# zhoupengwei/tloam

Hardware: AMD Instinct MI355X
Metric: gauss_newton_iters_per_sec (higher is better)
Workload: dtype f64

## Files before the change

tloam_amd/csrc/tl_api.hip:

```cpp
#include "tl_ctx.hpp"

using namespace tl;

extern "C" {

int tloam_abi_version(void) { return TLOAM_ABI_VERSION; }

const char* tloam_status_string(int s) {
  switch (s) {
    case TLOAM_OK: return "ok";
    case TLOAM_E_INVALID: return "invalid argument";
    case TLOAM_E_TOO_FEW_POINTS: return "fewer than 10 points in a feature cloud";
    case TLOAM_E_BAD_POSE: return "predicted pose is not a rigid transform";
    case TLOAM_E_HIP: return "HIP error / no gfx950 device";
    case TLOAM_E_RCCL: return "RCCL error";
    case TLOAM_E_NOT_READY: return "call sequence violated";
    case TLOAM_E_WEIGHT_RANGE: return "GNC weight outside [0,1]";
    default: return "unknown status";
  }
}

void tloam_default_config(tloam_tls_config* c) {
  if (!c) return;
  memset(c, 0, sizeof(*c));
// ... 29 lines not shown
  if (const char* e = getenv("TLOAM_DEBUG_MAX_SWEEPS")) c->dbg_max_sweeps = atoi(e);
  c->dbg_no_build_reuse = getenv("TLOAM_NO_BUILD_REUSE") != nullptr;
  c->dbg_no_eval_reuse = getenv("TLOAM_NO_EVAL_REUSE") != nullptr;
  c->no_device_loop = getenv("TLOAM_NO_DEVICE_LOOP") != nullptr;
  c->no_persistent_solve = getenv("TLOAM_NO_PERSISTENT_SOLVE") != nullptr;
  c->no_grid_ahead = getenv("TLOAM_NO_GRID_AHEAD") != nullptr;
  c->no_direct_set = getenv("TLOAM_NO_DIRECT_SET") != nullptr;
  c->no_qbin_ride = getenv("TLOAM_NO_QBIN_RIDE") != nullptr;
  if (const char* e = getenv("TLOAM_DEBUG_FAIL_HANDOVER")) c->dbg_fail_handover = atoi(e);
  {
    int cus = 0;
    if (hipDeviceGetAttribute(&cus, hipDeviceAttributeMultiprocessorCount, device_id) != hipSuccess) cus = 0;
    c->device_cus = cus;
  }
  c->fused_large = getenv("TLOAM_FUSED_LARGE") != nullptr;
  if (const char* e = getenv("TLOAM_PLANNED_SWEEPS")) c->dbg_planned_sweeps = atoi(e);
  memset(&c->stats, 0, sizeof(c->stats));
  constexpr size_t kBoxDoubles = (size_t)kKinds * 64 * 6 + 8;
  const unsigned flags = hipHostMallocMapped | hipHostMallocCoherent;
  const bool up = hipStreamCreateWithFlags(&c->stream, hipStreamNonBlocking) == hipSuccess &&
                  c->h_state.alloc(kMirrorSlots, flags) == hipSuccess && c->h_small.alloc(4096, hipHostMallocDefault) == hipSuccess &&
                  c->h_mirror.alloc(kMirrorSlots, flags) == hipSuccess && ((uintptr_t)c->h_mirror.h & 63u) == 0 &&
                  c->h_mirror.map() == hipSuccess && c->h_bbox.alloc(kBoxDoubles, flags) == hipSuccess &&
                  c->h_bbox.map() == hipSuccess && c->h_fault.alloc(kFaultWords, flags) == hipSuccess &&
                  c->h_fault.map() == hipSuccess;
  if (up) {
    c->h_state.zero();
    c->h_mirror.zero();
    c->h_bbox.zero();
    c->h_fault.zero();
  }
  if (!up || ensure_common(c) != TLOAM_OK) {
    (void)hipGetLastError();
    tloam_destroy(c);
    return TLOAM_E_HIP;
  }
  (void)hipMemsetAsync(c->state.p, 0, sizeof(GnState), c->stream);
  (void)hipMemsetAsync(c->seg_n.p, 0, 8 * sizeof(int), c->stream);
  (void)hipStreamSynchronize(c->stream);
  *out = c;
  return TLOAM_OK;
}

void tloam_destroy(tloam_ctx* c) {
  if (!c) return;
  (void)hipSetDevice(c->device);
  if (c->stream) (void)hipStreamSynchronize(c->stream);
  tlh::comm_release(c);
  tlh::loop_release(c);
  for (auto& e : c->ev_pool) (void)hipEventDestroy(e);
  for (hipEvent_t e : c->stage_ev)
    if (e) (void)hipEventDestroy(e);
// ... 81 lines not shown
```

tloam_amd/csrc/tl_api_frames.hip:

```cpp
#include <chrono>
#include "tl_ctx.hpp"

using namespace tl;

namespace tlh {
int wait_word(tloam_ctx* c, const unsigned long long* p, unsigned long long seq) {
  for (unsigned spins = 1;; ++spins) {
    if (__atomic_load_n(p, __ATOMIC_ACQUIRE) == seq) return TLOAM_OK;
    if ((spins & 0x7ffu) == 0) {
      const hipError_t e = hipStreamQuery(c->stream);
      if (e == hipSuccess) return __atomic_load_n(p, __ATOMIC_ACQUIRE) == seq ? TLOAM_OK : 1;
      if (e != hipErrorNotReady) HIPC(c, e);
    }
    __builtin_ia32_pause();
  }
}
int wait_segment(tloam_ctx* c, const unsigned long long* seg, unsigned long long number, unsigned long long payload[7]) {
  const unsigned long long seq = check_mix(number);
  for (unsigned spins = 1;; ++spins) {
    unsigned long long w[8], x = 0ull;
    for (int i = 0; i < 8; ++i) { w[i] = __atomic_load_n(seg + i, __ATOMIC_ACQUIRE); x ^= i < 7 ? tl::seg_word(w[i], i) : w[i]; }
    if (x == seq) {
      for (int i = 0; i < 7; ++i) payload[i] = w[i];
      return TLOAM_OK;
// ... 209 lines not shown
      const int rc = reserve_query_sort(c, out);
      if (rc != TLOAM_OK) return rc;
      frame->qbin->tile_of_slot = c->tile_of_slot.p;
      frame->qbin->rank_in_tile = c->tile_fill.p;
      frame->qbin->tile_cnt = c->tile_cnt.p;
      if (frame->fi.tile_cnt == c->tile_cnt.p) { qbin = frame->qbin; frame->qbin_done = true; }
    }
    launch_grid_scan_finalize_scatter_1p(gs, G.cell_cnt.p, nc + 1, G.cell_start.p, G.scan1p.p, c->h_fault.dev + kFaultScan1p, G.cell_of_pt.p,
                                         G.rank_of_pt.p, G.gp.p, c->stream, qbin, out);
    return TLOAM_OK;
  }
  const int tiles = scan_tiles_only(G.cell_cnt.p, G.cell_scan.p, nc + 1, G.scan_tmp.p, c->stream);
  if (tiles > 0) {
    launch_grid_finalize_scatter_all(gs, G.cell_scan.p, G.scan_tmp.p, tiles, G.cell_start.p, G.cell_cnt.p, G.cell_of_pt.p,
                                     G.rank_of_pt.p, G.gp.p, c->stream);
  } else {
    launch_exclusive_scan_u64(G.cell_cnt.p, G.cell_scan.p, nc + 1, G.scan_tmp.p, c->stream);
    launch_grid_finalize_all(gs, G.cell_scan.p, G.cell_start.p, G.cell_cnt.p, c->stream);
    launch_grid_scatter_all(gs, G.cell_of_pt.p, G.cell_scan.p, G.rank_of_pt.p, G.gp.p, c->stream);
  }
  return TLOAM_OK;
}
int build_grids(tloam_ctx* c, GridBuffers& G, const double radius[kKinds], GridView out[kKinds], FrameInitHook* frame) {
  CloudRef clouds[kKinds];
  bool known = true;
  for (int k = 0; k < kKinds; ++k) {
    const KindData& K = c->kd[k];
    clouds[k] = CloudRef{K.tx.p, K.ty.p, K.tz.p, K.tgt_set ? K.n_tgt : 0};
    if (radius[k] > 0.0 && clouds[k].n > 0 && !c->tgt_box_valid[k]) known = false;
  }
  return build_grids_over(c, G, radius, clouds, out, known ? c->tgt_box : nullptr, frame);
}
int enqueue_target_bounds(tloam_ctx* c) {
  GridSet gs;
  memset(&gs, 0, sizeof(gs));
  for (int k = 0; k < kKinds; ++k) {
    const KindData& K = c->kd[k];
    gs.tx[k] = K.tx.p; gs.ty[k] = K.ty.p; gs.tz[k] = K.tz.p;
    gs.n[k] = K.tgt_set ? (int)K.n_tgt : 0;
  }
  launch_bbox_all(gs, c->h_bbox.dev, c->stream);
  return TLOAM_OK;
}
void finish_target_bounds(tloam_ctx* c) {
  reduce_box_rows(c->h_bbox, c->tgt_box);
  for (int k = 0; k < kKinds; ++k) c->tgt_box_valid[k] = c->kd[k].tgt_set && c->kd[k].n_tgt > 0;
}
void exchange_clouds(tloam_ctx* c, FrameClouds& F) {
  for (int k = 0; k < kKinds; ++k) {
    KindData& K = c->kd[k];
    std::swap(K.n_src_full, F.n_src_full[k]); std::swap(K.src_lo, F.src_lo[k]); std::swap(K.n_src, F.n_src[k]);
    std::swap(K.n_tgt, F.n_tgt[k]);
    std::swap(K.src_aos, F.src_aos[k]); std::swap(K.tgt_aos, F.tgt_aos[k]);
    std::swap(K.src_ptr, F.src_ptr[k]);
    std::swap(K.tx, F.tx[k]); std::swap(K.ty, F.ty[k]); std::swap(K.tz, F.tz[k]);
    std::swap(K.src_set, F.src_set[k]); std::swap(K.tgt_set, F.tgt_set[k]);
    for (int a = 0; a < 6; ++a) std::swap(c->tgt_box[k][a], F.tgt_box[k][a]);
    std::swap(c->tgt_box_valid[k], F.tgt_box_valid[k]);
    K.grid_valid = false;
  }
  c->grids_ahead = false; c->tgt_gen++;
  std::swap(c->src_pack, F.src_pack);
  c->have_build = false;
}
int source_frame_reserve(tloam_ctx* c, const size_t n[4], size_t cnt4[4]) {
  size_t lo4[kKinds], hi4[kKinds];
  tloam_shard_ranges_frame(n, c->rank, c->nranks, lo4, hi4);
  for (int k = 0; k < kKinds; ++k) {
    KindData& K = c->kd[k];
// ... 65 lines not shown
  K.tgt_set = true;
  return TLOAM_OK;
}
}

int tloam_set_source(tloam_ctx* c, int kind, const double* xyz, size_t n) {
  if (!c) return TLOAM_E_INVALID;
  HIPC(c, hipSetDevice(c->device));
  const int rc = set_source_async(c, kind, xyz, n);
  if (rc != TLOAM_OK) return rc;
  HIPC(c, hipStreamSynchronize(c->stream));
  return TLOAM_OK;
}

int tloam_set_target(tloam_ctx* c, int kind, const double* xyz, size_t n) {
  if (!c) return TLOAM_E_INVALID;
  HIPC(c, hipSetDevice(c->device));
  return tlh::set_target_copy(c, kind, xyz, n, hipMemcpyHostToDevice);
}

int tloam_set_source_frame(tloam_ctx* c, const double* const xyz[4], const size_t n[4]) {
  if (!c || !xyz || !n) return TLOAM_E_INVALID;
  HIPC(c, hipSetDevice(c->device));
  return set_source_frame_packed(c, xyz, n);
}

int tloam_set_target_frame(tloam_ctx* c, const double* const xyz[4], const size_t n[4]) {
  if (!c || !xyz || !n) return TLOAM_E_INVALID;
  for (int k = 0; k < kKinds; ++k)
    if ((n[k] > 0 && !xyz[k]) || n[k] > kMaxPoints) return TLOAM_E_INVALID;
  HIPC(c, hipSetDevice(c->device));
  return tlh::set_target_frame_from(c, xyz, n, hipMemcpyHostToDevice);
}
}

namespace tlh {
int set_target_frame_from(tloam_ctx* c, const double* const xyz[4], const size_t n[4], hipMemcpyKind from) {
  int rc = TLOAM_OK;
  for (int k = 0; k < kKinds && rc == TLOAM_OK; ++k) rc = set_target_async(c, k, xyz[k], n[k], false, from);
  if (rc == TLOAM_OK) {
    IngestArgs A;
    for (int k = 0; k < kKinds; ++k) {
      KindData& K = c->kd[k];
      A.aos[k] = K.tgt_aos.p; A.x[k] = K.tx.p; A.y[k] = K.ty.p; A.z[k] = K.tz.p;
      A.n[k] = (int)K.n_tgt;
    }
    launch_ingest_targets(A, c->h_bbox.dev, c->stream);
  }
  HIPC(c, hipStreamSynchronize(c->stream));
  if (rc == TLOAM_OK) finish_target_bounds(c);
  if (rc == TLOAM_OK && one_rank(c) && !c->no_grid_ahead) {
    double radius[kKinds];
    GridView views[kKinds];
    bool all = true;
    for (int k = 0; k < kKinds; ++k) { radius[k] = kind_radius(c->cfg, k); all = all && c->tgt_box_valid[k]; }
    if (all) {
      rc = build_grids(c, c->grids_next, radius, views, nullptr);
      if (rc == TLOAM_OK) {
        for (int k = 0; k < kKinds; ++k) c->gv_next[k] = views[k];
        c->grids_ahead = true;
        c->grids_next_gen = c->tgt_gen;
      }
    }
  }
  return rc;
}
}

extern "C" {

int tloam_frame_stash(tloam_ctx* c, int slot) {
  if (!c || slot < 0 || slot > (1 << 20)) return TLOAM_E_INVALID;
  if (c->active) return TLOAM_E_NOT_READY;
  HIPC(c, hipSetDevice(c->device));
  if ((size_t)slot >= c->frame_store.size()) c->frame_store.resize((size_t)slot + 1);
  if (c->frame_selected == slot) {
    exchange_clouds(c, *c->frame_store[slot]);
    c->frame_selected = -1;
    return TLOAM_OK;
  }
  if (c->frame_selected >= 0) return TLOAM_E_NOT_READY;
  if (!c->frame_store[slot]) {
    c->frame_store[slot].reset(new (std::nothrow) FrameClouds());
    if (!c->frame_store[slot]) return TLOAM_E_INVALID;
  } else {
    HIPC(c, hipStreamSynchronize(c->stream));
    *c->frame_store[slot] = FrameClouds();
  }
// ... 28 lines not shown
```

tloam_amd/csrc/tl_api_match.hip:

```cpp
#include <atomic>
#include <chrono>

#include "tl_ctx.hpp"

using namespace tl;

namespace {
int sync_stream(tloam_ctx* c) {
  HIPC(c, hipStreamSynchronize(c->stream));
  return TLOAM_OK;
}
}

namespace tlh {
int reserve_seg(tloam_ctx* c, int k, size_t n) {
  KindData& K = c->kd[k];
  const size_t cap = round_up(std::max<size_t>(n, 1), kChunk) + kChunk;
  HIPC(c, K.c_idx.reserve(cap));
  if (cap > K.c_stride) {
    const size_t stride = std::max(cap, K.c_stride + K.c_stride / 2);
    HIPC(c, K.c_buf.reserve(stride * kSegStreams));
    K.c_stride = stride;
  }
  K.c_cap = cap - kChunk;
// ... 352 lines not shown
    GridView gviews[kKinds];
    for (int k = 0; k < kKinds; ++k) gviews[k] = c->kd[k].gv;
    const size_t ntiles = (size_t)build_tile_count(gviews, c->sv.slot_off);
    HIPC(c, c->tile_cnt.reserve(ntiles + 1 > c->tile_cnt.cap ? 2 * ntiles + 64 : ntiles + 1));
    hook.fi.tile_cnt = c->tile_cnt.p;
    hook.fi.n_tile_cnt = (int)ntiles + 1;
    launch_frame_init(hook.fi, hook.b, c->stream);
  }
  if (c->direct) {
    bool all = true;
    for (int k = 0; k < kKinds; ++k) all = all && c->kd[k].gv.n > 0;
    if (!all) {
      c->direct = false;
      HIPC(c, hipMemsetAsync(c->seg_n.p, 0, kKinds * sizeof(int), c->stream));
    }
  }
  c->wait_us = 0.0;
  c->mu = 1.0;
  c->noise_bound_sq = c->cfg.noise_bound * c->cfg.noise_bound;
  if (c->noise_bound_sq < 1e-16) c->noise_bound_sq = 1e-2;
  for (int k = 0; k < kKinds; ++k) { c->prev_cost[k] = INFINITY; c->cur_cost[k] = INFINITY; }
  c->iter = 0;
  c->active = true;
  c->have_build = false;
  memset(&c->stats, 0, sizeof(c->stats));
  memcpy(c->stats.se3, x, sizeof(x));
  c->ev_used = 0;
  c->ev_batch_idx.clear();
  c->batch_launches = 0;
  return TLOAM_OK;
}

namespace {
constexpr int kMaxOuterFast = kMirrorSlots;

void outer_params(const tloam_ctx* c, BuildParams* bp, GridView grids[kKinds]) {
  for (int k = 0; k < kKinds; ++k) {
    bp->radius[k] = kind_radius(c->cfg, k);
    bp->maxnum[k] = kind_maxnum(c->cfg, k);
    bp->active[k] = kind_active(c->cfg, k);
    grids[k] = c->kd[k].gv;
  }
  bp->edge_dir_thres = c->cfg.edge_dir_thres;
}
int outer_reserve(tloam_ctx* c, const GridView grids[kKinds]) { return tlh::reserve_query_sort(c, grids); }
}
// ... 1046 lines not shown
```

tloam_amd/csrc/tl_api_submap.hip:

```cpp
#include "tl_ctx.hpp"

using namespace tl;

extern "C" {

void tloam_submap_default_config(tloam_submap_config* cfg) {
  if (!cfg) return;
  cfg->planar_frame_size = 3;
  cfg->sphere_frame_size = 3;
  cfg->edge_crop_box_length = 100.0;
  cfg->ground_crop_box_length = 100.0;
  cfg->edge_down_sample_submap = 0.3;
  cfg->ground_down_sample_submap = 0.45;
  cfg->ground_down_sample = 0.3;
}

namespace {
int submap_reserve_work(tloam_ctx* c, size_t n) {
  SubmapState& S = c->submap;
  const size_t m = std::max<size_t>(n, 1), cap = voxel_table_size(m);
  HIPC(c, S.min_partial.reserve(256 * 6)); HIPC(c, S.vmin.reserve(8)); HIPC(c, S.counts.reserve(8));
  if (!S.overflow.p) {
    HIPC(c, S.overflow.reserve(8));
    HIPC(c, hipMemsetAsync(S.overflow.p, 0, 8 * sizeof(int), c->stream));
// ... 34 lines not shown
  J.mask = voxel_table_size(std::max<size_t>(n, 1)) - 1;
  W.min_partial = S.min_partial.p; W.vmin = S.vmin.p;
  W.keys = S.keys.p; W.cnt = S.cnt.p; W.off = S.off.p;
  W.slot_of_pt = S.slot_of_pt.p; W.urank = S.urank.p; W.members = S.members.p; W.sorted = S.sorted.p;
  W.leader = S.leader.p; W.leader_scan = S.leader_scan.p; W.scan_tmp = S.scan_tmp.p; W.overflow = S.overflow.p;
  W.n_out = S.counts.p;
  W.host_seg = &c->h_mirror.dev[kMirrorSlots - 1].w[0];
  W.host_seq = ++c->mirror_seq;
  W.use_ticket = (c->vox_ticket || (long long)(n + 256) / 256 > (long long)vox_emit_resident_blocks(c->device_cus)) ? 1 : 0;
  W.fault = c->h_fault.dev + kFaultVoxEmit;
  S.pending_seq = W.host_seq;
  *Jout = J;
  *Wout = W;
  return TLOAM_OK;
}
int submap_crop_voxel(tloam_ctx* c, const CropVoxelSeg seg[2], int nseg) {
  VoxelJob J;
  VoxelWork W;
  const int rc = submap_job(c, seg, nseg, &J, &W);
  if (rc != TLOAM_OK) return rc;
  launch_crop_voxel(J, W, c->stream);
  return TLOAM_OK;
}
int submap_upload(tloam_ctx* c, const double* xyz, size_t n, hipMemcpyKind from = hipMemcpyHostToDevice) {
  SubmapState& S = c->submap;
  HIPC(c, S.in_aos.reserve(3 * std::max<size_t>(n, 1)));
  if (n > 0) HIPC(c, hipMemcpyAsync(S.in_aos.p, xyz, sizeof(double) * 3 * n, from, c->stream));
  return TLOAM_OK;
}
int submap_finish(tloam_ctx* c, size_t* n_edge, size_t* n_ground) {
  SubmapState& S = c->submap;
  unsigned long long h[2] = {0, 0};
  int ov = 0;
  bool have = false;
  if (S.pending_seq) {
    const unsigned long long* seg = &c->h_mirror[kMirrorSlots - 1].w[0];
    unsigned long long pay[7];
    const int rc = wait_segment(c, seg, S.pending_seq, pay);
    if (rc < 0) return rc;
    if (rc == TLOAM_OK) { h[0] = pay[0]; h[1] = pay[1]; ov = (int)pay[2]; have = true; }
    S.pending_seq = 0ull;
  }
  if (!have) {
    HIPC(c, hipMemcpyAsync(h, S.counts.p, sizeof(h), hipMemcpyDeviceToHost, c->stream));
    HIPC(c, hipMemcpyAsync(&ov, S.overflow.p, sizeof(int), hipMemcpyDeviceToHost, c->stream));
    HIPC(c, hipStreamSynchronize(c->stream));
// ... 16 lines not shown
  if (!c || (n_planar && !planar) || (n_sphere && !sphere) || (n_edge && !edge) || (n_ground && !ground) ||
      n_planar > kMaxPoints || n_sphere > kMaxPoints || n_edge > kMaxPoints || n_ground > kMaxPoints)
    return TLOAM_E_INVALID;
  HIPC(c, hipSetDevice(c->device));
  const tloam_submap_config want = cfg_or_default(cfg, tloam_submap_default_config);
  if (!tlh::submap_config_ok(want))
    return TLOAM_E_INVALID;
  return tlh::submap_init_body(c, want, planar, n_planar, sphere, n_sphere, edge, n_edge, ground, n_ground, hipMemcpyHostToDevice);
}

}

namespace tlh {
bool submap_config_ok(const tloam_submap_config& want) {
  return want.planar_frame_size >= 1 && want.sphere_frame_size >= 1 && want.edge_down_sample_submap > 0.0 &&
         want.ground_down_sample_submap > 0.0 && want.ground_down_sample > 0.0;
}

int submap_init_body(tloam_ctx* c, const tloam_submap_config& want, const double* planar, size_t n_planar, const double* sphere,
                     size_t n_sphere, const double* edge, size_t n_edge, const double* ground, size_t n_ground, hipMemcpyKind from) {
  SubmapState& S = c->submap;
  S = SubmapState();
  S.cfg = want;
  int rc = set_target_copy(c, TLOAM_KIND_EDGE, edge, n_edge, from);
  if (rc == TLOAM_OK) rc = set_target_copy(c, TLOAM_KIND_PLANAR, planar, n_planar, from);
  if (rc == TLOAM_OK) rc = set_target_copy(c, TLOAM_KIND_SPHERE, sphere, n_sphere, from);
  if (rc != TLOAM_OK) return rc;
  rc = submap_upload(c, ground, n_ground, from);
  if (rc != TLOAM_OK) return rc;
  const size_t m = std::max<size_t>(n_ground, 1);
  HIPC(c, S.wx.reserve(m)); HIPC(c, S.wy.reserve(m)); HIPC(c, S.wz.reserve(m));
  launch_aos_to_soa(S.in_aos.p, n_ground, S.wx.p, S.wy.p, S.wz.p, c->stream);
  rc = submap_reserve_work(c, n_ground);
  if (rc != TLOAM_OK) return rc;
  {
    const CropVoxelSeg seg[2] = {{TLOAM_KIND_GROUND, n_ground, kNoLo, kNoHi, S.cfg.ground_down_sample},
                                 {TLOAM_KIND_GROUND, 0, kNoLo, kNoHi, S.cfg.ground_down_sample}};
    rc = submap_crop_voxel(c, seg, 1);
  }
  if (rc != TLOAM_OK) return rc;
  size_t ne = 0, ng = 0;
  rc = submap_finish(c, &ne, &ng);
  if (rc != TLOAM_OK) return rc;
  (void)ng;
  c->kd[TLOAM_KIND_GROUND].n_tgt = ne;
  c->kd[TLOAM_KIND_GROUND].tgt_set = true;
  c->tgt_box_valid[TLOAM_KIND_GROUND] = false;
  c->grids_ahead = false; c->tgt_gen++;
  S.inited = true;
  return TLOAM_OK;
}
}

static int submap_update_body(tloam_ctx* c, const double pose[16], const double* planar, size_t n_planar,
                              const double* sphere, size_t n_sphere, const double* edge, size_t n_edge,
                              const double* ground, size_t n_ground, DBuf<double>* resident = nullptr);

extern "C" {

int tloam_submap_update(tloam_ctx* c, const double pose[16], const double* planar, size_t n_planar,
                        const double* sphere, size_t n_sphere, const double* edge, size_t n_edge,
                        const double* ground, size_t n_ground) {
  if (!c || !pose || (n_planar && !planar) || (n_sphere && !sphere) || (n_edge && !edge) || (n_ground && !ground) ||
      n_planar > kMaxPoints || n_sphere > kMaxPoints || n_edge > kMaxPoints || n_ground > kMaxPoints)
    return TLOAM_E_INVALID;
  if (!c->submap.inited) return TLOAM_E_NOT_READY;
  for (int i = 0; i < 16; ++i)
    if (!(pose[i] - pose[i] == 0.0)) return TLOAM_E_BAD_POSE;
  HIPC(c, hipSetDevice(c->device));
  const int rc = submap_update_body(c, pose, planar, n_planar, sphere, n_sphere, edge, n_edge, ground, n_ground);
  if (rc != TLOAM_OK) (void)hipStreamSynchronize(c->stream);
  return rc;
// ... 1 lines not shown

}

namespace tlh {
int submap_update_resident(tloam_ctx* c, const double pose[16], size_t n_planar, size_t n_sphere, size_t n_edge, size_t n_ground,
                           DBuf<double>& block) {
  if (!c->submap.inited) return TLOAM_E_NOT_READY;
  for (int i = 0; i < 16; ++i)
    if (!(pose[i] - pose[i] == 0.0)) return TLOAM_E_BAD_POSE;
  const int rc = submap_update_body(c, pose, nullptr, n_planar, nullptr, n_sphere, nullptr, n_edge, nullptr, n_ground, &block);
  if (rc != TLOAM_OK) (void)hipStreamSynchronize(c->stream);
  return rc;
}
}

extern "C" {

static int submap_update_body(tloam_ctx* c, const double pose[16], const double* planar, size_t n_planar,
                              const double* sphere, size_t n_sphere, const double* edge, size_t n_edge,
                              const double* ground, size_t n_ground, DBuf<double>* resident) {
  SubmapState& S = c->submap;
  (void)sphere;
  bool fused_front = false;
  for (int k = 0; k < kKinds; ++k) c->tgt_box_valid[k] = false;
  c->grids_ahead = false; c->tgt_gen++;
  const bool in_place = S.cfg.planar_frame_size <= transform_ring_max();
  const double* stage_view = nullptr;
  size_t stage_off[3] = {0, 0, 0};
  int stage_half = -1;
  auto push = [&](std::vector<std::unique_ptr<RingFrame>>& ring, const double* xyz, size_t n, int keep, bool upload) -> int {
    std::unique_ptr<RingFrame> fresh;
    if ((int)ring.size() >= keep) {
      fresh = std::move(ring.front());
      ring.erase(ring.begin());
      while ((int)ring.size() >= keep) ring.erase(ring.begin());
    } else {
      fresh.reset(new RingFrame());
    }
    ring.push_back(std::move(fresh));
    RingFrame* const f = ring.back().get();
    f->n = n;
    memcpy(f->pose, pose, sizeof(double) * 16);
    if (!upload) return TLOAM_OK;
    const double* parts[3] = {xyz, edge, ground};
    const size_t counts[3] = {3 * n, 3 * n_edge, 3 * n_ground};
    if (resident) {
// ... 95 lines not shown
      size_t ring_max = 0;
      const double* aos[16]; size_t nn[16]; const double* poses[16];
      int cnt = 0;
      for (const auto& f : S.planar_ring) { aos[cnt] = f->aos.p; nn[cnt] = f->n; poses[cnt] = f->pose; ring_max = std::max(ring_max, f->n); ++cnt; }
      if (stage_view) aos[cnt - 1] = stage_view + stage_off[0];
      const size_t rows = submap_front_rows(ring_max, std::max(n_in[0], n_in[1]));
      if (S.min_partial.cap < rows * 6) HIPC(c, hipStreamSynchronize(c->stream));
      HIPC(c, S.min_partial.reserve(rows * 6));
      VoxelJob J;
      VoxelWork W;
      rc = submap_job(c, seg, 2, &J, &W);
      if (rc != TLOAM_OK) return rc;
      KindData& P = c->kd[TLOAM_KIND_PLANAR];
      KindData& Q = c->kd[TLOAM_KIND_SPHERE];
      launch_submap_front(cnt, aos, nn, poses, A, J, W, P.tx.p, P.ty.p, P.tz.p, Q.tx.p, Q.ty.p, Q.tz.p, S.wx.p, S.wy.p, S.wz.p, c->stream,
                          cnt - 1, stage_view ? S.planar_ring.back()->aos.p : nullptr);
      launch_crop_voxel(J, W, c->stream, true);
    } else {
      launch_assemble(A, S.wx.p, S.wy.p, S.wz.p, c->stream);
      rc = submap_crop_voxel(c, seg, 2);
      if (rc != TLOAM_OK) return rc;
    }
  }
  size_t ne = 0, ng = 0;
  rc = submap_finish(c, &ne, &ng);
  if (stage_view) (void)tlh::stage_release(c, stage_half, true);
  if (rc != TLOAM_OK) return rc;
  c->kd[TLOAM_KIND_EDGE].n_tgt = ne;
  c->kd[TLOAM_KIND_GROUND].n_tgt = ng;
  c->kd[TLOAM_KIND_EDGE].tgt_set = c->kd[TLOAM_KIND_GROUND].tgt_set = true;
  return TLOAM_OK;
}

}

namespace tlh {
int voxel_down_sample_launch(tloam_ctx* c, const size_t n[2], const double voxel[2], int nseg, double* const out[2][3]) {
  const CropVoxelSeg seg[2] = {{TLOAM_KIND_EDGE, n[0], kNoLo, kNoHi, voxel[0]},
                               {TLOAM_KIND_GROUND, nseg > 1 ? n[1] : 0, kNoLo, kNoHi, voxel[nseg > 1 ? 1 : 0]}};
  VoxelJob J;
  VoxelWork W;
  const int rc = submap_job(c, seg, nseg, &J, &W, out);
  if (rc != TLOAM_OK) return rc;
  W.host_seg = nullptr;
  c->submap.pending_seq = 0ull;
  launch_crop_voxel(J, W, c->stream);
  return TLOAM_OK;
}
}

extern "C" {

int tloam_voxel_down_sample(tloam_ctx* c, double voxel, const double* xyz, size_t n, double* out, size_t capacity,
// ... 51 lines not shown
```

tloam_amd/csrc/tl_common.hpp:

```cpp
#pragma once
#include <cstddef>

#include <hip/hip_runtime.h>
#include <stdint.h>

#include "../../include/tloam_hip.h"
#include "tl_se3.hpp"

namespace tl {

constexpr int kKinds = 4;
constexpr int kAccN = 28;
constexpr int kAccStride = 32;
constexpr int kReduceBuf = 48;
constexpr int kChunk = 128;
constexpr int kMaxK = 8;
constexpr int kMaxRanks = 16;

__host__ __device__ inline int res_type_of_kind(int kind) {
  return kind == TLOAM_KIND_EDGE ? TLOAM_RES_LINE : (kind == TLOAM_KIND_SPHERE ? TLOAM_RES_POINT : TLOAM_RES_PLANE);
}

struct GridView {
  const double4* gp;
// ... 204 lines not shown
  for (int i = block * 256 + (int)threadIdx.x; i < fi.n_tile_cnt; i += nblocks * 256) fi.tile_cnt[i] = 0ull;
  if (block == 0) {
    constexpr int kWords = (int)(sizeof(GnState) / sizeof(double));
    for (int i = threadIdx.x; i < kWords; i += 256) reinterpret_cast<double*>(b.st)[i] = 0.0;
    if (threadIdx.x < 8)
      b.seg_n[threadIdx.x] = (fi.direct && threadIdx.x < kKinds) ? fi.slot_off[threadIdx.x + 1] - fi.slot_off[threadIdx.x] : 0;
    if (threadIdx.x == 0) b.flags[n] = 0ull;
    __syncthreads();
    if (threadIdx.x == 0) {
      GnState* st = b.st;
#pragma unroll
      for (int i = 0; i < 6; ++i) st->x[i] = fi.x[i];
      st->T_cur = se3_exp(st->x);
      st->no_eval_reuse = fi.no_eval_reuse;
      st->prev_planar = __builtin_inf();
      st->run_build = 1;
      arm_solver(*st);
    }
  }
}
#endif
void launch_frame_init(const FrameInit& fi, const FrameInitBufs& b, hipStream_t s);
void launch_bbox_all(const GridSet& gs, double* out , hipStream_t s);
void launch_grid_count_all(const GridSet& gs, unsigned long long* cell_cnt, int* cell_of_pt, int* rank_of_pt,
                           hipStream_t s, const FrameInitHook* frame = nullptr);
void launch_grid_finalize_all(const GridSet& gs, const unsigned long long* cell_scan, int* cell_start,
                              unsigned long long* cell_cnt , hipStream_t s);
int scan_tiles_only(const unsigned long long* in, unsigned long long* out, size_t n, unsigned long long* totals, hipStream_t s,
                    const int* gate = nullptr);
void launch_grid_finalize_scatter_all(const GridSet& gs, const unsigned long long* cell_scan, const unsigned long long* totals,
                                      int tiles, int* cell_start, unsigned long long* cell_cnt, const int* cell_of_pt,
                                      const int* rank_of_pt, double4* gp, hipStream_t s);
void launch_grid_scatter_all(const GridSet& gs, const int* cell_of_pt, const unsigned long long* cell_scan,
                             const int* rank_of_pt, double4* gp, hipStream_t s);
size_t scan_1p_ctl_elems(size_t n);
bool scan_1p_applies(size_t n, int device_cus);
void launch_scan_counts_1p(const unsigned long long* in, unsigned long long* out, size_t n, unsigned long long* ctl, unsigned* fault,
                           hipStream_t s);
void launch_grid_scan_finalize_scatter_1p(const GridSet& gs, unsigned long long* cell_cnt, size_t ncells_plus_1, int* cell_start,
                                          unsigned long long* ctl, unsigned* fault, const int* cell_of_pt, const int* rank_of_pt, double4* gp,
                                          hipStream_t s, const QueryBinRide* qbin = nullptr, const GridView* views = nullptr);

void launch_build(const SlotView& sv, const GridView grids[kKinds], const BuildParams& bp, GnState* st,
                  int* tile_of_slot, unsigned long long* tile_cnt, unsigned long long* tile_scan, int* tile_fill,
                  double4* qrec, unsigned long long* scan_tmp, bool rebin, hipStream_t s, const int* gate = nullptr,
                  unsigned long long* scan1p_ctl = nullptr, unsigned* scan1p_fault = nullptr, const CorrView* direct_cv = nullptr,
// ... 36 lines not shown
  unsigned* fault;
};
size_t voxel_table_size(size_t n);
int vox_emit_resident_blocks(int device_cus);
void launch_transform_to_soa(const double* aos, size_t n, const double M[16], double* ox, double* oy, double* oz,
                             hipStream_t s);
void launch_transform_to_soa2(const double* aos, size_t n, const double M[16], double* ax, double* ay, double* az,
                              double* bx, double* by, double* bz, hipStream_t s);
struct AssembleArgs {
  const double *ox[2], *oy[2], *oz[2];
  const double* aos[2];
  size_t n_old[2], n_new[2], base[2];
  double M[16];
};
void launch_assemble(const AssembleArgs& A, double* wx, double* wy, double* wz, hipStream_t s);
int transform_ring_max();
void launch_transform_ring(int count, const double* const aos[], const size_t n[], const double* const poses[],
                           double* ax, double* ay, double* az, double* bx, double* by, double* bz, hipStream_t s);
void launch_copy3(const double* ax, const double* ay, const double* az, size_t n, double* ox, double* oy, double* oz,
                  hipStream_t s);
void launch_soa_to_aos(const double* x, const double* y, const double* z, size_t n, double* aos, hipStream_t s);
void launch_blit_doubles(const double* src_host_view, double* dst, size_t n, hipStream_t s);
void launch_crop_voxel(const VoxelJob& J, const VoxelWork& W, hipStream_t s, bool front_done = false);
size_t submap_front_rows(size_t n_ring_max, size_t n_seg_max);
void launch_submap_front(int count, const double* const aos[], const size_t n[], const double* const poses[], const AssembleArgs& A,
                         const VoxelJob& J, const VoxelWork& W, double* px, double* py, double* pz, double* qx, double* qy, double* qz,
                         double* wx, double* wy, double* wz, hipStream_t s, int copy_frame = -1, double* copy_dst = nullptr);

struct GatherJob {
  const double *sx, *sy, *sz;
  double *dx, *dy, *dz;
  const int* idx1;
  const int* idx2;
  const int* count;
  int n;
  int n1, src_n;
  int ss, ds;
};
constexpr int kGatherMaxJobs = 8;
struct GatherArgs { GatherJob j[kGatherMaxJobs]; };
void launch_gather_lists(const GatherArgs& A, int jobs, hipStream_t s);
struct OdomCountArgs {
  const unsigned long long* total;
  const double* ranked;
  int planar_num, sphere_num;
  double planar_scan_thres, cvr_scan;
// ... 501 lines not shown
```

tloam_amd/csrc/tl_ctx.hpp:

```cpp
#pragma once

#include <dlfcn.h>
#include <math.h>
#include <stdio.h>
#include <stdlib.h>
#include <string.h>

#include <algorithm>
#include <initializer_list>
#include <memory>
#include <new>
#include <string>
#include <utility>
#include <vector>

#include "tl_common.hpp"
#include "tl_seg.hpp"


namespace tlh {
using namespace tl;


template <class T>
// ... 416 lines not shown
struct tloam_ctx {
  tloam_tls_config cfg;
  SubmapState submap;
  FeatBuffers feat;
  SegBuffers seg;
  OdomState odom;
  MapState map;
  VmapState vmap;
  DeskewState deskew;
  PlaceState place;
  LoopState loop;
  GraphState graph;
  CmapState cmap;
  int device = 0;
  hipStream_t stream = nullptr;
  KindData kd[kKinds];
  DBuf<double> sx, sy, sz, w_src, raw;
  DBuf<double> fit_x, fit_y, fit_z;
  DBuf<unsigned long long> flags, scan, scan_tmp, tile_cnt, tile_scan;
  DBuf<unsigned long long> scan1p_q;
  bool scan1p_q_use = false;
  bool grids_ahead = false;
  unsigned long long tgt_gen = 0, grids_next_gen = ~0ull;
  bool no_grid_ahead = false;
  bool no_scan_1p = false;
  DBuf<unsigned char> flagb;
  DBuf<double> fin_rows;
  bool fused_large = false;
  DBuf<int> tile_of_slot, tile_fill;
  DBuf<double4> qrec;
  GridBuffers grids;
  GridBuffers grids_next;
  tl::GridView gv_next[tl::kKinds];
  SlotView sv{};
  CorrView cv{};
  DBuf<int> seg_n;
  DBuf<double> partials, red48, sums16, wpart, rank_counts, se3_dev, bbox_dev, misc;
  DBuf<GnState> state;
  Pinned<GnState> h_state;
  Pinned<double> h_small;
  int k3_grid = 1;
  bool k3_single = false;
  bool k3_wide = false;
  int dbg_max_sweeps = 0;
  bool dbg_no_build_reuse = false;
  bool dbg_no_eval_reuse = false;
  bool no_device_loop = false;
  bool no_persistent_solve = false;
  bool hand_over_timed_out = false;
  int dbg_fail_handover = 0;
  int device_cus = 0;
  Pinned<double> h_bbox;
  double tgt_box[tl::kKinds][6];
  bool tgt_box_valid[tl::kKinds] = {false, false, false, false};
  double wait_us = 0.0;
  double hs[8] = {0, 0, 0, 0, 0, 0, 0, 0};
  long hs_n = 0;
  double hs_exit = 0.0;
  double hs_entry = 0.0;
  Pinned<tl::MirrorSlot> h_mirror;
  unsigned long long mirror_seq = 0;
  Pinned<unsigned> h_fault;
  bool scan1p_retried = false;
  bool vox_ticket = false;
  DBuf<double> src_pack;
  Pinned<double> h_stage[2];
  hipEvent_t stage_ev[2] = {nullptr, nullptr};
  bool stage_busy[2] = {false, false};
  int stage_next = 0;
  std::vector<std::unique_ptr<tlh::FrameClouds>> frame_store;
  int frame_selected = -1;
  int dbg_planned_sweeps = 0;
  std::vector<int> planned_sweeps;
  bool prebuilt = false;
  int rank = 0, nranks = 1;
// ... 348 lines not shown
int cmap_side_range(const tloam_ctx* c, bool ran, size_t first, size_t count);
int deskew_frame_upload(tloam_ctx* c, const double* t_sec, size_t n, tloam_odom_stats* st);
int deskew_frame_launch(tloam_ctx* c, size_t n, unsigned long long* bad_host, tloam_odom_stats* st);
void deskew_frame_end(tloam_ctx* c, bool accepted, int64_t frame);
inline const double* frame_scan(const tloam_ctx* c) { return c->deskew.active ? c->deskew.aos.p : c->seg.aos.p; }
int place_frame_reserve(tloam_ctx* c, size_t n);
void place_frame_end(tloam_ctx* c, bool accepted, int64_t frame, const double pose[16], const double* scan, size_t n);
bool place_clouds_on(const tloam_ctx* c);
int place_clouds_reserve(tloam_ctx* c, const size_t n[8]);
void place_clouds_note(tloam_ctx* c, const tl::LoopSpan spans[8]);
int arena_grow(tloam_ctx* c, size_t need_doubles);
void loop_release(tloam_ctx* c);
void graph_correct_pose(const tloam_ctx* c, size_t keyframe, const double pose_in[16], double pose_out[16]);
int set_target_frame_from(tloam_ctx* c, const double* const xyz[4], const size_t n[4], hipMemcpyKind from);
int voxel_down_sample_launch(tloam_ctx* c, const size_t n[2], const double voxel[2], int nseg, double* const out[2][3]);
int build_grids_over(tloam_ctx* c, GridBuffers& G, const double radius[tl::kKinds], const CloudRef clouds[tl::kKinds],
                     tl::GridView out[tl::kKinds], const double (*known_boxes)[6] = nullptr,
                     tl::FrameInitHook* frame = nullptr);
int build_grids(tloam_ctx* c, GridBuffers& G, const double radius[tl::kKinds], tl::GridView out[tl::kKinds],
                tl::FrameInitHook* frame = nullptr);
void reduce_box_rows(const double* box_rows, double boxes[tl::kKinds][6]);
int enqueue_target_bounds(tloam_ctx* c);
void finish_target_bounds(tloam_ctx* c);
}
```

tloam_amd/csrc/tl_nn.hip:

```cpp
#include <string.h>
#include <algorithm>
#include <atomic>

#include "tl_common.hpp"
#include "tl_knn.hpp"
#include "tl_finish.hpp"

namespace tl {

__global__ void k_aos_to_soa(const double* __restrict__ aos, size_t n, double* __restrict__ x,
                             double* __restrict__ y, double* __restrict__ z) {
  size_t i = (size_t)blockIdx.x * blockDim.x + threadIdx.x;
  const size_t stride = (size_t)gridDim.x * blockDim.x;
  for (; i < n; i += stride) {
    x[i] = aos[3 * i];
    y[i] = aos[3 * i + 1];
    z[i] = aos[3 * i + 2];
  }
}
void launch_aos_to_soa(const double* aos, size_t n, double* x, double* y, double* z, hipStream_t s) {
  if (n == 0) return;
  int blocks = (int)((n + 255) / 256);
  if (blocks > 4096) blocks = 4096;
  hipLaunchKernelGGL(k_aos_to_soa, dim3(blocks), dim3(256), 0, s, aos, n, x, y, z);
// ... 383 lines not shown
    lo[0] = fmin(lo[0], a); hi[0] = fmax(hi[0], a);
    lo[1] = fmin(lo[1], b); hi[1] = fmax(hi[1], b);
    lo[2] = fmin(lo[2], c); hi[2] = fmax(hi[2], c);
  }
#pragma unroll
  for (int off = 32; off > 0; off >>= 1) {
#pragma unroll
    for (int a = 0; a < 3; ++a) {
      lo[a] = fmin(lo[a], __shfl_down(lo[a], off, 64));
      hi[a] = fmax(hi[a], __shfl_down(hi[a], off, 64));
    }
  }
  const int lane = threadIdx.x & 63, wave = threadIdx.x >> 6;
  if (lane == 0) {
#pragma unroll
    for (int a = 0; a < 3; ++a) { red[wave][a] = lo[a]; red[wave][3 + a] = hi[a]; }
  }
  __syncthreads();
  if (threadIdx.x < 6) {
    double v = red[0][threadIdx.x];
    for (int w = 1; w < 4; ++w) v = (threadIdx.x < 3) ? fmin(v, red[w][threadIdx.x]) : fmax(v, red[w][threadIdx.x]);
    out[((size_t)k * gridDim.x + blockIdx.x) * 6 + threadIdx.x] = v;
  }
}
void launch_ingest_targets(const IngestArgs& A, double* out, hipStream_t s) {
  hipLaunchKernelGGL(k_ingest_targets, dim3(64, kKinds), dim3(256), 0, s, A, out);
}
void launch_bbox_all(const GridSet& gs, double* out, hipStream_t s) {
  hipLaunchKernelGGL(k_bbox_all, dim3(64, kKinds), dim3(256), 0, s, gs, out);
}


__global__ __launch_bounds__(256) void k_grid_count_all(GridSet gs, unsigned long long* __restrict__ cell_cnt,
                                                        int* __restrict__ cell_of_pt, int* __restrict__ rank_of_pt,
                                                        FrameInit fi, FrameInitBufs fb) {
  const int k = blockIdx.y;
  if (k == kKinds) {
    frame_init_body(fi, fb, (int)blockIdx.x, (int)gridDim.x);
    return;
  }
  const int n = gs.n[k];
  for (int i = blockIdx.x * blockDim.x + threadIdx.x; i < n; i += gridDim.x * blockDim.x) {
    const int cx = clampi(cell_coord(gs.tx[k][i], gs.org[k][0], gs.inv_cell[k], gs.dim[k][0]), 0, gs.dim[k][0] - 1);
    const int cy = clampi(cell_coord(gs.ty[k][i], gs.org[k][1], gs.inv_cell[k], gs.dim[k][1]), 0, gs.dim[k][1] - 1);
    const int cz = clampi(cell_coord(gs.tz[k][i], gs.org[k][2], gs.inv_cell[k], gs.dim[k][2]), 0, gs.dim[k][2] - 1);
    const int c = (cz * gs.dim[k][1] + cy) * gs.dim[k][0] + cx;
// ... 939 lines not shown
```

tloam_amd/csrc/tl_submap.hip:

```cpp
#include <atomic>
#include <algorithm>
#include <string.h>

#include "tl_voxel.hpp"

namespace tl {

namespace {
struct Mat16 { double m[16]; };

__global__ void k_transform_to_soa(const double* __restrict__ aos, size_t n, Mat16 M, double* __restrict__ ox,
                                   double* __restrict__ oy, double* __restrict__ oz) {
  const size_t i = (size_t)blockIdx.x * blockDim.x + threadIdx.x;
  if (i >= n) return;
  const double x = aos[3 * i], y = aos[3 * i + 1], z = aos[3 * i + 2];
  double r[4];
#pragma unroll
  for (int a = 0; a < 4; ++a) r[a] = ((M.m[a] * x + M.m[4 + a] * y) + M.m[8 + a] * z) + M.m[12 + a] * 1.0;
  ox[i] = r[0] / r[3];
  oy[i] = r[1] / r[3];
  oz[i] = r[2] / r[3];
}

__global__ void k_transform_to_soa2(const double* __restrict__ aos, size_t n, Mat16 M, double* __restrict__ ax,
// ... 427 lines not shown
    int occ = 0;
    if (hipOccupancyMaxActiveBlocksPerMultiprocessor(&occ, k_vox_emit, 256, 0) != hipSuccess || occ < 1) { (void)hipGetLastError(); occ = 1; }
    per_cu = occ;
    per_cu_cache.store(occ, std::memory_order_relaxed);
  }
  const long long all = (long long)device_cus * per_cu;
  return (int)(all - all / 16);
}
size_t voxel_table_size(size_t n) {
  size_t cap = 1024;
  while (cap < 2 * n) cap <<= 1;
  return cap;
}

void launch_crop_voxel(const VoxelJob& J, const VoxelWork& W, hipStream_t s, bool front_done) {
  const size_t n = J.n;
  constexpr int kMinBlocks = 256;
  const int emit_blocks = (int)blocks_for(n + 1);
  if (!front_done) hipLaunchKernelGGL(k_vox_min2, dim3(kMinBlocks), dim3(256), 0, s, J, W, emit_blocks);
  if (n > 0) hipLaunchKernelGGL(k_vox_insert2, dim3(blocks_for(n)), dim3(256), 0, s, J, W);
  hipLaunchKernelGGL(k_vox_emit, dim3(emit_blocks), dim3(256), 0, s, J, W, emit_blocks);
}

}
```

Measured before the change: 62320.

## Compute submap target bounds on device during update to enable grid prebuild

Submap update paths now launch a counted bounding-box kernel and a ready-flag post right after the voxel step, recording a pending sequence. At the next source-frame set, the host waits on that flag, reduces the boxes, and enqueues the ahead-of-time grid build for the new target generation. The aim is to keep grids prebuilt after submap updates, instead of leaving them invalidated and rebuilding synchronously during matching. It adds a pinned buffer, extra launches, generation tracking and a host wait on a mirrored segment.

```diff
diff --git a/tloam_amd/csrc/tl_api.hip b/tloam_amd/csrc/tl_api.hip
--- a/tloam_amd/csrc/tl_api.hip
+++ b/tloam_amd/csrc/tl_api.hip
@@ -75,12 +75,14 @@
                   c->h_state.alloc(kMirrorSlots, flags) == hipSuccess && c->h_small.alloc(4096, hipHostMallocDefault) == hipSuccess &&
                   c->h_mirror.alloc(kMirrorSlots, flags) == hipSuccess && ((uintptr_t)c->h_mirror.h & 63u) == 0 &&
                   c->h_mirror.map() == hipSuccess && c->h_bbox.alloc(kBoxDoubles, flags) == hipSuccess &&
-                  c->h_bbox.map() == hipSuccess && c->h_fault.alloc(kFaultWords, flags) == hipSuccess &&
+                  c->h_bbox.map() == hipSuccess && c->h_bbox_next.alloc(kBoxDoubles, flags) == hipSuccess &&
+                  c->h_bbox_next.map() == hipSuccess && c->h_fault.alloc(kFaultWords, flags) == hipSuccess &&
                   c->h_fault.map() == hipSuccess;
   if (up) {
     c->h_state.zero();
     c->h_mirror.zero();
     c->h_bbox.zero();
+    c->h_bbox_next.zero();
     c->h_fault.zero();
   }
   if (!up || ensure_common(c) != TLOAM_OK) {
diff --git a/tloam_amd/csrc/tl_api_frames.hip b/tloam_amd/csrc/tl_api_frames.hip
--- a/tloam_amd/csrc/tl_api_frames.hip
+++ b/tloam_amd/csrc/tl_api_frames.hip
@@ -255,6 +255,7 @@
   return TLOAM_OK;
 }
 int build_grids(tloam_ctx* c, GridBuffers& G, const double radius[kKinds], GridView out[kKinds], FrameInitHook* frame) {
+  take_pending_bounds(c);
   CloudRef clouds[kKinds];
   bool known = true;
   for (int k = 0; k < kKinds; ++k) {
@@ -275,9 +276,19 @@
   launch_bbox_all(gs, c->h_bbox.dev, c->stream);
   return TLOAM_OK;
 }
+static void bounds_from_rows(tloam_ctx* c, const double* rows) {
+  reduce_box_rows(rows, c->tgt_box);
+  for (int k = 0; k < kKinds; ++k) c->tgt_box_valid[k] = c->kd[k].tgt_set && c->kd[k].n_tgt > 0;
+}
 void finish_target_bounds(tloam_ctx* c) {
-  reduce_box_rows(c->h_bbox, c->tgt_box);
-  for (int k = 0; k < kKinds; ++k) c->tgt_box_valid[k] = c->kd[k].tgt_set && c->kd[k].n_tgt > 0;
+  bounds_from_rows(c, c->h_bbox);
+}
+void take_pending_bounds(tloam_ctx* c) {
+  const unsigned long long seq = std::exchange(c->bounds_seq, 0ull);
+  if (!seq || c->bounds_gen != c->tgt_gen) return;
+  unsigned long long pay[7];
+  if (wait_segment(c, bounds_ready_seg(c->h_mirror.h), seq, pay) != TLOAM_OK) return;
+  bounds_from_rows(c, c->h_bbox_next);
 }
 void exchange_clouds(tloam_ctx* c, FrameClouds& F) {
   for (int k = 0; k < kKinds; ++k) {
@@ -389,6 +400,12 @@
 int tloam_set_source_frame(tloam_ctx* c, const double* const xyz[4], const size_t n[4]) {
   if (!c || !xyz || !n) return TLOAM_E_INVALID;
   HIPC(c, hipSetDevice(c->device));
+  if (c->ahead_wanted_gen == c->tgt_gen && !c->active) {
+    c->ahead_wanted_gen = ~0ull;
+    tlh::take_pending_bounds(c);
+    const int rc = tlh::enqueue_grids_ahead(c);
+    if (rc != TLOAM_OK) return rc;
+  }
   return set_source_frame_packed(c, xyz, n);
 }
 
@@ -416,21 +433,23 @@
   }
   HIPC(c, hipStreamSynchronize(c->stream));
   if (rc == TLOAM_OK) finish_target_bounds(c);
-  if (rc == TLOAM_OK && one_rank(c) && !c->no_grid_ahead) {
-    double radius[kKinds];
-    GridView views[kKinds];
-    bool all = true;
-    for (int k = 0; k < kKinds; ++k) { radius[k] = kind_radius(c->cfg, k); all = all && c->tgt_box_valid[k]; }
-    if (all) {
-      rc = build_grids(c, c->grids_next, radius, views, nullptr);
-      if (rc == TLOAM_OK) {
-        for (int k = 0; k < kKinds; ++k) c->gv_next[k] = views[k];
-        c->grids_ahead = true;
-        c->grids_next_gen = c->tgt_gen;
-      }
-    }
-  }
+  if (rc == TLOAM_OK) rc = enqueue_grids_ahead(c);
   return rc;
+}
+int enqueue_grids_ahead(tloam_ctx* c) {
+  if (!grids_ahead_on(c)) return TLOAM_OK;
+  double radius[kKinds];
+  GridView views[kKinds];
+  for (int k = 0; k < kKinds; ++k) {
+    if (!c->tgt_box_valid[k]) return TLOAM_OK;
+    radius[k] = kind_radius(c->cfg, k);
+  }
+  const int rc = build_grids(c, c->grids_next, radius, views, nullptr);
+  if (rc != TLOAM_OK) return rc;
+  for (int k = 0; k < kKinds; ++k) c->gv_next[k] = views[k];
+  c->grids_ahead = true;
+  c->grids_next_gen = c->tgt_gen;
+  return TLOAM_OK;
 }
 }
 
diff --git a/tloam_amd/csrc/tl_api_match.hip b/tloam_amd/csrc/tl_api_match.hip
--- a/tloam_amd/csrc/tl_api_match.hip
+++ b/tloam_amd/csrc/tl_api_match.hip
@@ -398,6 +398,7 @@
   for (int k = 0; k < kKinds; ++k) { c->prev_cost[k] = INFINITY; c->cur_cost[k] = INFINITY; }
   c->iter = 0;
   c->active = true;
+  c->matched_since_update = true;
   c->have_build = false;
   memset(&c->stats, 0, sizeof(c->stats));
   memcpy(c->stats.se3, x, sizeof(x));
diff --git a/tloam_amd/csrc/tl_api_submap.hip b/tloam_amd/csrc/tl_api_submap.hip
--- a/tloam_amd/csrc/tl_api_submap.hip
+++ b/tloam_amd/csrc/tl_api_submap.hip
@@ -80,6 +80,25 @@
   launch_crop_voxel(J, W, c->stream);
   return TLOAM_OK;
 }
+unsigned long long submap_bounds_launch(tloam_ctx* c, const size_t cap[kKinds], const unsigned long long* const dev_n[kKinds]) {
+  GridSet gs;
+  memset(&gs, 0, sizeof(gs));
+  BoxCounts dn;
+  for (int k = 0; k < kKinds; ++k) {
+    const KindData& K = c->kd[k];
+    gs.tx[k] = K.tx.p; gs.ty[k] = K.ty.p; gs.tz[k] = K.tz.p;
+    gs.n[k] = (int)cap[k];
+    dn.n[k] = dev_n[k];
+  }
+  const unsigned long long seq = ++c->mirror_seq;
+  launch_bbox_counted(gs, dn, c->h_bbox_next.dev, c->stream);
+  launch_post_ready(tlh::bounds_ready_seg(c->h_mirror.dev), seq, c->stream);
+  return seq;
+}
+void submap_bounds_pending(tloam_ctx* c, unsigned long long seq) {
+  c->bounds_seq = seq;
+  c->bounds_gen = c->ahead_wanted_gen = c->tgt_gen;
+}
 int submap_upload(tloam_ctx* c, const double* xyz, size_t n, hipMemcpyKind from = hipMemcpyHostToDevice) {
   SubmapState& S = c->submap;
   HIPC(c, S.in_aos.reserve(3 * std::max<size_t>(n, 1)));
@@ -142,6 +161,7 @@
   SubmapState& S = c->submap;
   S = SubmapState();
   S.cfg = want;
+  c->matched_since_update = false;
   int rc = set_target_copy(c, TLOAM_KIND_EDGE, edge, n_edge, from);
   if (rc == TLOAM_OK) rc = set_target_copy(c, TLOAM_KIND_PLANAR, planar, n_planar, from);
   if (rc == TLOAM_OK) rc = set_target_copy(c, TLOAM_KIND_SPHERE, sphere, n_sphere, from);
@@ -153,12 +173,21 @@
   launch_aos_to_soa(S.in_aos.p, n_ground, S.wx.p, S.wy.p, S.wz.p, c->stream);
   rc = submap_reserve_work(c, n_ground);
   if (rc != TLOAM_OK) return rc;
+  const bool ahead = grids_ahead_on(c);
   {
     const CropVoxelSeg seg[2] = {{TLOAM_KIND_GROUND, n_ground, kNoLo, kNoHi, S.cfg.ground_down_sample},
                                  {TLOAM_KIND_GROUND, 0, kNoLo, kNoHi, S.cfg.ground_down_sample}};
     rc = submap_crop_voxel(c, seg, 1);
   }
   if (rc != TLOAM_OK) return rc;
+  unsigned long long bounds = 0ull;
+  if (ahead) {
+    size_t cap[kKinds];
+    const unsigned long long* dev_n[kKinds] = {nullptr, nullptr, nullptr, nullptr};
+    for (int k = 0; k < kKinds; ++k) cap[k] = k == TLOAM_KIND_GROUND ? n_ground : c->kd[k].n_tgt;
+    dev_n[TLOAM_KIND_GROUND] = S.counts.p;
+    bounds = submap_bounds_launch(c, cap, dev_n);
+  }
   size_t ne = 0, ng = 0;
   rc = submap_finish(c, &ne, &ng);
   if (rc != TLOAM_OK) return rc;
@@ -168,6 +197,7 @@
   c->tgt_box_valid[TLOAM_KIND_GROUND] = false;
   c->grids_ahead = false; c->tgt_gen++;
   S.inited = true;
+  if (ahead) submap_bounds_pending(c, bounds);
   return TLOAM_OK;
 }
 }
@@ -215,6 +245,8 @@
   SubmapState& S = c->submap;
   (void)sphere;
   bool fused_front = false;
+  const bool ahead = tlh::grids_ahead_on(c) && c->matched_since_update;
+  c->matched_since_update = false;
   for (int k = 0; k < kKinds; ++k) c->tgt_box_valid[k] = false;
   c->grids_ahead = false; c->tgt_gen++;
   const bool in_place = S.cfg.planar_frame_size <= transform_ring_max();
@@ -356,6 +388,14 @@
       if (rc != TLOAM_OK) return rc;
     }
   }
+  unsigned long long bounds = 0ull;
+  if (ahead) {
+    size_t cap[kKinds];
+    const unsigned long long* dev_n[kKinds] = {nullptr, nullptr, nullptr, nullptr};
+    cap[TLOAM_KIND_PLANAR] = cap[TLOAM_KIND_SPHERE] = total;
+    for (int s = 0; s < 2; ++s) { cap[accs[s].kind] = n_in[s]; dev_n[accs[s].kind] = S.counts.p + s; }
+    bounds = submap_bounds_launch(c, cap, dev_n);
+  }
   size_t ne = 0, ng = 0;
   rc = submap_finish(c, &ne, &ng);
   if (stage_view) (void)tlh::stage_release(c, stage_half, true);
@@ -363,6 +403,7 @@
   c->kd[TLOAM_KIND_EDGE].n_tgt = ne;
   c->kd[TLOAM_KIND_GROUND].n_tgt = ng;
   c->kd[TLOAM_KIND_EDGE].tgt_set = c->kd[TLOAM_KIND_GROUND].tgt_set = true;
+  if (ahead) submap_bounds_pending(c, bounds);
   return TLOAM_OK;
 }
 
diff --git a/tloam_amd/csrc/tl_common.hpp b/tloam_amd/csrc/tl_common.hpp
--- a/tloam_amd/csrc/tl_common.hpp
+++ b/tloam_amd/csrc/tl_common.hpp
@@ -250,6 +250,10 @@
 #endif
 void launch_frame_init(const FrameInit& fi, const FrameInitBufs& b, hipStream_t s);
 void launch_bbox_all(const GridSet& gs, double* out , hipStream_t s);
+struct BoxCounts {
+  const unsigned long long* n[kKinds];
+};
+void launch_bbox_counted(const GridSet& gs, const BoxCounts& dn, double* out , hipStream_t s);
 void launch_grid_count_all(const GridSet& gs, unsigned long long* cell_cnt, int* cell_of_pt, int* rank_of_pt,
                            hipStream_t s, const FrameInitHook* frame = nullptr);
 void launch_grid_finalize_all(const GridSet& gs, const unsigned long long* cell_scan, int* cell_start,
@@ -332,6 +336,7 @@
 void launch_soa_to_aos(const double* x, const double* y, const double* z, size_t n, double* aos, hipStream_t s);
 void launch_blit_doubles(const double* src_host_view, double* dst, size_t n, hipStream_t s);
 void launch_crop_voxel(const VoxelJob& J, const VoxelWork& W, hipStream_t s, bool front_done = false);
+void launch_post_ready(unsigned long long* host_seg, unsigned long long host_seq, hipStream_t s);
 size_t submap_front_rows(size_t n_ring_max, size_t n_seg_max);
 void launch_submap_front(int count, const double* const aos[], const size_t n[], const double* const poses[], const AssembleArgs& A,
                          const VoxelJob& J, const VoxelWork& W, double* px, double* py, double* pz, double* qx, double* qy, double* qz,
diff --git a/tloam_amd/csrc/tl_ctx.hpp b/tloam_amd/csrc/tl_ctx.hpp
--- a/tloam_amd/csrc/tl_ctx.hpp
+++ b/tloam_amd/csrc/tl_ctx.hpp
@@ -462,6 +462,8 @@
   bool scan1p_q_use = false;
   bool grids_ahead = false;
   unsigned long long tgt_gen = 0, grids_next_gen = ~0ull;
+  unsigned long long bounds_seq = 0, bounds_gen = 0, ahead_wanted_gen = ~0ull;
+  bool matched_since_update = false;
   bool no_grid_ahead = false;
   bool no_scan_1p = false;
   DBuf<unsigned char> flagb;
@@ -491,6 +493,7 @@
   int dbg_fail_handover = 0;
   int device_cus = 0;
   Pinned<double> h_bbox;
+  Pinned<double> h_bbox_next;
   double tgt_box[tl::kKinds][6];
   bool tgt_box_valid[tl::kKinds] = {false, false, false, false};
   double wait_us = 0.0;
@@ -885,4 +888,8 @@
 void reduce_box_rows(const double* box_rows, double boxes[tl::kKinds][6]);
 int enqueue_target_bounds(tloam_ctx* c);
 void finish_target_bounds(tloam_ctx* c);
-}
+inline bool grids_ahead_on(const tloam_ctx* c) { return one_rank(c) && !c->no_grid_ahead; }
+int enqueue_grids_ahead(tloam_ctx* c);
+void take_pending_bounds(tloam_ctx* c);
+inline unsigned long long* bounds_ready_seg(tl::MirrorSlot* slots) { return &slots[kMirrorSlots - 1].w[8]; }
+}
diff --git a/tloam_amd/csrc/tl_nn.hip b/tloam_amd/csrc/tl_nn.hip
--- a/tloam_amd/csrc/tl_nn.hip
+++ b/tloam_amd/csrc/tl_nn.hip
@@ -429,6 +429,50 @@
     for (int w = 1; w < 4; ++w) v = (threadIdx.x < 3) ? fmin(v, red[w][threadIdx.x]) : fmax(v, red[w][threadIdx.x]);
     out[((size_t)k * gridDim.x + blockIdx.x) * 6 + threadIdx.x] = v;
   }
+}
+__global__ __launch_bounds__(256) void k_bbox_counted(GridSet gs, BoxCounts dn, double* __restrict__ out) {
+  __shared__ double red[4][6];
+  const int k = blockIdx.y;
+  const double* __restrict__ x = gs.tx[k];
+  const double* __restrict__ y = gs.ty[k];
+  const double* __restrict__ z = gs.tz[k];
+  int n = gs.n[k];
+  if (dn.n[k]) {
+    const unsigned long long m = *dn.n[k];
+    n = m < (unsigned long long)n ? (int)m : n;
+  }
+  double lo[3] = {1e300, 1e300, 1e300}, hi[3] = {-1e300, -1e300, -1e300};
+  for (int i = blockIdx.x * 256 + threadIdx.x; i < n; i += gridDim.x * 256) {
+    double a = x[i], b = y[i], c = z[i];
+    if (!(fabs(a) < __builtin_inf())) a = __builtin_nan("");
+    if (!(fabs(b) < __builtin_inf())) b = __builtin_nan("");
+    if (!(fabs(c) < __builtin_inf())) c = __builtin_nan("");
+    lo[0] = fmin(lo[0], a); hi[0] = fmax(hi[0], a);
+    lo[1] = fmin(lo[1], b); hi[1] = fmax(hi[1], b);
+    lo[2] = fmin(lo[2], c); hi[2] = fmax(hi[2], c);
+  }
+#pragma unroll
+  for (int off = 32; off > 0; off >>= 1) {
+#pragma unroll
+    for (int a = 0; a < 3; ++a) {
+      lo[a] = fmin(lo[a], __shfl_down(lo[a], off, 64));
+      hi[a] = fmax(hi[a], __shfl_down(hi[a], off, 64));
+    }
+  }
+  const int lane = threadIdx.x & 63, wave = threadIdx.x >> 6;
+  if (lane == 0) {
+#pragma unroll
+    for (int a = 0; a < 3; ++a) { red[wave][a] = lo[a]; red[wave][3 + a] = hi[a]; }
+  }
+  __syncthreads();
+  if (threadIdx.x < 6) {
+    double v = red[0][threadIdx.x];
+    for (int w = 1; w < 4; ++w) v = (threadIdx.x < 3) ? fmin(v, red[w][threadIdx.x]) : fmax(v, red[w][threadIdx.x]);
+    out[((size_t)k * gridDim.x + blockIdx.x) * 6 + threadIdx.x] = v;
+  }
+}
+void launch_bbox_counted(const GridSet& gs, const BoxCounts& dn, double* out, hipStream_t s) {
+  hipLaunchKernelGGL(k_bbox_counted, dim3(64, kKinds), dim3(256), 0, s, gs, dn, out);
 }
 void launch_ingest_targets(const IngestArgs& A, double* out, hipStream_t s) {
   hipLaunchKernelGGL(k_ingest_targets, dim3(64, kKinds), dim3(256), 0, s, A, out);
diff --git a/tloam_amd/csrc/tl_submap.hip b/tloam_amd/csrc/tl_submap.hip
--- a/tloam_amd/csrc/tl_submap.hip
+++ b/tloam_amd/csrc/tl_submap.hip
@@ -473,4 +473,14 @@
   hipLaunchKernelGGL(k_vox_emit, dim3(emit_blocks), dim3(256), 0, s, J, W, emit_blocks);
 }
 
-}
+namespace {
+__global__ __launch_bounds__(64) void k_post_ready(unsigned long long* host_seg, unsigned long long host_seq) {
+  const int tid = (int)threadIdx.x;
+  if (tid < 8) post_host_segment(host_seg, host_seq, 0ull, tid);
+}
+}
+void launch_post_ready(unsigned long long* host_seg, unsigned long long host_seq, hipStream_t s) {
+  hipLaunchKernelGGL(k_post_ready, dim3(1), dim3(64), 0, s, host_seg, host_seq);
+}
+
+}
```

After: 61710. About the same (-1.0%).
